# ZackHodari/morgana

Measured on AMD Instinct MI355X. Metric: acoustic frames/sec (fwd+bwd+step), F0Model 600->1, batch 256x1000, higher is better.
Workload: dtype bf16

## Files before the change

### morgana_amd/csrc/gemm_bf16_big.hip

```cpp
#include "common.h"
#include "phone_front.h"
#include "expand_reduce.h"

#include <type_traits>

typedef __bf16 bfv8 __attribute__((ext_vector_type(8)));
typedef __bf16 bfv4 __attribute__((ext_vector_type(4)));


#define MG_ZERO_ELEMS 16384
__device__ uint16_t g_zero_row[MG_ZERO_ELEMS];

__device__ __forceinline__ void glds16(const uint16_t* src, unsigned char* lds_wave_base) {
    const unsigned lds_off = (unsigned)(unsigned long long)((__attribute__((address_space(3))) unsigned char*)lds_wave_base);
    const unsigned lds_uni = __builtin_amdgcn_readfirstlane(lds_off);
    unsigned keep;
    asm volatile("s_mov_b32 %0, m0\n\ts_mov_b32 m0, %2\n\ts_nop 0\n\tglobal_load_lds_dwordx4 %1, off\n\ts_mov_b32 m0, %0"
                 : "=&s"(keep)
                 : "v"(src), "s"(lds_uni)
                 : "memory");
}


#define WAIT_VM_BARRIER(N) asm volatile("s_waitcnt vmcnt(" #N ")\n\ts_barrier" ::: "memory")
#define WAIT_LGKM_BARRIER() asm volatile("s_waitcnt lgkmcnt(0)\n\ts_barrier" ::: "memory")

MG_STAMP_DECL(g_stamps_nt);

#define NT_BIG_LDS(BN_) (((BN_) == 256 ? 4 : 6) * (256 * 64 + (BN_) * 64))
template <int BN, int EPI, int X3 = 0>
__device__ __forceinline__ void gemm_nt_big_body(unsigned char* __restrict__ smem, const unsigned block_id, const uint16_t* __restrict__ A,
                                                 int lda, const int32_t* __restrict__ rows, int64_t M, int K, const uint16_t* __restrict__ Bm,
                                                 int ldb, int N, const float* __restrict__ bias_in, const uint16_t* __restrict__ H, int ldh,
                                                 const int32_t* __restrict__ h_rows, void* __restrict__ Cv_in, int ldc, int tiles_m, int tiles_n,
                                                 int c_f32, float* __restrict__ colsum = nullptr, int wt = 0) {
    const float* bias = bias_in;
    void* Cv = Cv_in;
    constexpr int BM = 256;
    constexpr int WAVES_N = BN / 64;
    constexpr int WAVES_M = 8 / WAVES_N;
    constexpr int WM = BM / WAVES_M;
    constexpr int TM = WM / 32, TN = 2;
    constexpr int A_BYTES = BM * 64, B_BYTES = BN * 64;
    constexpr int STAGE = A_BYTES + B_BYTES;
    constexpr int GA = BM / 16 / 8;
    constexpr int GB = BN / 16 / 8;
    constexpr int NL = GA + GB;
    constexpr int NS = (BN == 256) ? 4 : 6;

    static_assert(NS * STAGE == NT_BIG_LDS(BN), "LDS size helper");

    unsigned tile_id = block_id;
    int my_pass = 0;
    if (X3 == 2) {
        const unsigned per_pass = (unsigned)((tiles_m + 7) / 8) * 8u * (unsigned)tiles_n;
        my_pass = (int)(block_id / per_pass);
        tile_id = block_id - (unsigned)my_pass * per_pass;
    }
    const int xcd = tile_id & 7, jj = tile_id >> 3;
    const int tile_n = jj % tiles_n;
    const int tile_m = (jj / tiles_n) * 8 + xcd;
    if (tile_m >= tiles_m) return;

    const int tid = threadIdx.x, lane = tid & 63;
    const int wave = __builtin_amdgcn_readfirstlane(tid >> 6);
#ifdef MG_STAMPS
    unsigned long long ts0, ts1 = 0, ts2, ts3, tr0, tr1, ta, tb, sum_wait = 0, sum_issue = 0;
    MG_STAMP(ts0);
    MG_STAMP_REAL(tr0);
#endif
    const int wm0 = (wave / WAVES_N) * WM, wn0 = (wave % WAVES_N) * 64;
    const int64_t m0 = (int64_t)tile_m * BM;
    const int n0 = tile_n * BN;
    const int n_kp = (K + 31) / 32;
    const int n_kt = X3 == 1 ? 3 * n_kp : n_kp;
    const int a_lo = lda >> 1, b_lo = ldb >> 1;
    if (X3 == 2) {
        if (my_pass > 0) bias = nullptr;
        Cv = reinterpret_cast<float*>(Cv) + (size_t)my_pass * (size_t)M * ldc;
    }

    const uint16_t* asrc[GA];
    const uint16_t* bsrc[GB];
#pragma unroll
    for (int i = 0; i < GA; ++i) {
        const int row = (wave * GA + i) * 16 + (lane >> 2);
        const int c = (lane & 3) ^ ((row >> 2) & 3);
        const int64_t m = m0 + row;
        const uint16_t* p = g_zero_row;
        if (m < M) {
            if (rows) {
                const int r = rows[m];
                if (r >= 0) p = A + (size_t)r * lda;
            } else {
                p = A + (size_t)m * lda;
            }
        }
        asrc[i] = p + c * 8;
    }
#pragma unroll
    for (int i = 0; i < GB; ++i) {
        const int row = (wave * GB + i) * 16 + (lane >> 2);
        const int c = (lane & 3) ^ ((row >> 2) & 3);
        const int n = n0 + row;
        bsrc[i] = (n < N ? Bm + (size_t)n * ldb : g_zero_row) + c * 8;
    }

    auto issue = [&](int kt) {
        unsigned char* st = smem + (kt % NS) * STAGE;
        int ka = kt * 32, kb = kt * 32;
        if (X3) {
            const int pass = X3 == 2 ? my_pass : kt % 3, w = (X3 == 2 ? kt : kt / 3) * 32;
            ka = w + (pass == 2 ? a_lo : 0);
            kb = w + (pass == 1 ? b_lo : 0);
        }
#pragma unroll
        for (int i = 0; i < GA; ++i) glds16(asrc[i] + ka, st + (wave * GA + i) * 1024);
#pragma unroll
        for (int i = 0; i < GB; ++i) glds16(bsrc[i] + kb, st + A_BYTES + (wave * GB + i) * 1024);
    };

    f32x16 acc[TM][TN];
#pragma unroll
    for (int i = 0; i < TM; ++i)
#pragma unroll
        for (int j = 0; j < TN; ++j)
#pragma unroll
            for (int r = 0; r < 16; ++r) acc[i][j][r] = 0.f;

    const int lr = lane & 31, lh = lane >> 5;
    int aoff[TM], boff[TN];
#pragma unroll
    for (int i = 0; i < TM; ++i) {
        const int row = wm0 + i * 32 + lr;
        aoff[i] = row * 64 + ((lh ^ ((row >> 2) & 3)) << 4);
    }
#pragma unroll
    for (int j = 0; j < TN; ++j) {
        const int row = wn0 + j * 32 + lr;
        boff[j] = A_BYTES + row * 64 + ((lh ^ ((row >> 2) & 3)) << 4);
    }

#pragma unroll
    for (int p = 0; p < NS - 1; ++p)
// ... 697 lines not shown
                    }
                    const bfv2 h01 = bfv2{(__bf16)v[0], (__bf16)v[1]}, h23 = bfv2{(__bf16)v[2], (__bf16)v[3]};
                    const u32x2_t pk = u32x2_t{__builtin_bit_cast(unsigned int, h01), __builtin_bit_cast(unsigned int, h23)};
                    if (X3) {
                        const bfv2 l01 = bfv2{(__bf16)(v[0] - (float)h01[0]), (__bf16)(v[1] - (float)h01[1])};
                        const bfv2 l23 = bfv2{(__bf16)(v[2] - (float)h23[0]), (__bf16)(v[3] - (float)h23[1])};
                        pk_lo[X3 ? j : 0][q] = u32x2_t{__builtin_bit_cast(unsigned int, l01), __builtin_bit_cast(unsigned int, l23)};
                    }
                    const int chunk = 4 * j + q;
                    *reinterpret_cast<u32x2_t*>(patch + lr * SP + ((chunk ^ (lr & 7)) << 4) + 8 * lh) = pk;
                }
            store_rows(i, 0);
            if (X3) {
#pragma unroll
                for (int j = 0; j < TN; ++j)
#pragma unroll
                    for (int q = 0; q < 4; ++q)
                        *reinterpret_cast<u32x2_t*>(patch + lr * SP + (((4 * j + q) ^ (lr & 7)) << 4) + 8 * lh) = pk_lo[X3 ? j : 0][q];
                store_rows(i, ldc >> 1);
            }
        }
        MG_STAMP(tb);
        MG_STAMP_ADD(sum_epi, tb, ta);
    }
    };
    if (lag) run_tiles(std::true_type{}); else run_tiles(std::false_type{});
#ifdef MG_STAMPS
    MG_STAMP(ts2);
    asm volatile("s_waitcnt vmcnt(0)" ::: "memory");
    MG_STAMP(ts3);
    MG_STAMP_REAL(tr1);
    const int sb = block_id;
    MG_STAMP_STORE(g_stamps_ntp, sb, wave, lane, 0, ts0);
    MG_STAMP_STORE(g_stamps_ntp, sb, wave, lane, 1, ts1);
    MG_STAMP_STORE(g_stamps_ntp, sb, wave, lane, 2, ts2);
    MG_STAMP_STORE(g_stamps_ntp, sb, wave, lane, 3, ts3);
    MG_STAMP_STORE(g_stamps_ntp, sb, wave, lane, 4, tr0);
    MG_STAMP_STORE(g_stamps_ntp, sb, wave, lane, 5, tr1);
    MG_STAMP_STORE(g_stamps_ntp, sb, wave, lane, 6, sum_wait);
    MG_STAMP_STORE(g_stamps_ntp, sb, wave, lane, 7, sum_epi);
#endif
}

template <int BN, int EPI, bool STAG, int BK, int MODE = 0>
__global__ __launch_bounds__(512) void gemm_nt_persist_kernel(const uint16_t* __restrict__ A, int lda, const int32_t* __restrict__ rows,
                                                              int64_t M, int K, const uint16_t* __restrict__ Bm, int ldb, int N,
                                                              const float* __restrict__ bias, uint16_t* __restrict__ C, int ldc,
                                                              int tiles_m, int tiles_n, int probe) {
    __shared__ __attribute__((aligned(16))) unsigned char smem[ntp_lds_bytes<BN, BK, MODE>()];
    gemm_nt_persist_body<BN, EPI, STAG, BK, MODE>(smem, blockIdx.x, gridDim.x, A, lda, rows, M, K, Bm, ldb, N, bias, C, ldc, tiles_m, tiles_n,
                                                  probe);
}

template <int EPI, int BMV = 256, int X3 = 0, int BK = 32>
__global__ __launch_bounds__(512) void phone_front_gemm_kernel(unsigned side_blocks, int wave_ints, PhoneFrontArgs pf, const uint16_t* __restrict__ A, int lda,
                                                               int64_t M, int K, const uint16_t* __restrict__ Bm, int ldb, int N,
                                                               const float* __restrict__ bias, uint16_t* __restrict__ C, int ldc, int tiles_m,
                                                               int tiles_n, int wt) {
    static_assert(ntp_lds_bytes<256, BK, 0>() == ntp_lds_bytes<256, 32, 0>(), "the front's jobs were sized for this LDS block");
    __shared__ __attribute__((aligned(16))) unsigned char smem[ntp_lds_bytes<256, BK, 0>()];
    if (blockIdx.x < side_blocks) {
        if (pf.lds_ints > 0) {
            if (wave_ints > 0)
                phone_front_wave_jobs(pf, (int)blockIdx.x * 8 + (int)(threadIdx.x >> 6), (int)side_blocks * 8,
                                      reinterpret_cast<int*>(smem) + (threadIdx.x >> 6) * wave_ints);
            else
                phone_front_block<512>(pf, blockIdx.x, side_blocks, reinterpret_cast<int*>(smem));
        }
        return;
    }
    if (pf.probe & 8) return;
    gemm_nt_persist_body<256, EPI, false, BK, 0, BMV, X3>(smem, blockIdx.x - side_blocks, gridDim.x - side_blocks, A, lda, nullptr, M, K, Bm, ldb, N, bias, C,
                                                     ldc, tiles_m, tiles_n, 0, wt);
}

#define WG_ROWS_MAX 4096
#define WG_STAGES(TKW_) (((TKW_) == 5 || (TKW_) == 4) ? 4 : 3)
MG_STAMP_DECL(g_stamps_wg);

#define WG_BIG_PX(TKW_) ((64 * (TKW_) * 2 + 255) / 256 * 256)
#define WG_BIG_LDS(TKW_) (WG_STAGES(TKW_) * (32 * 256 + 32 * WG_BIG_PX(TKW_)) + WG_ROWS_MAX * 4)
#define WG_STAGES_NW(TKW_, NW_) (((NW_) == 2 && (TKW_) == 5) ? 3 : WG_STAGES(TKW_))
#define WG_BIG_LDS_NW(TKW_, NW_) (WG_STAGES_NW(TKW_, NW_) * (32 * 256 * (NW_) + 32 * WG_BIG_PX(TKW_)) + WG_ROWS_MAX * 4)
template <int TKW, bool DYR = false, int NW = 1, int X3 = 0, bool WT = false>
__device__ __forceinline__ void wgrad_big_body(unsigned char* __restrict__ smem, const unsigned block_id, const uint16_t* __restrict__ dY,
                                               int lddy, const uint16_t* __restrict__ A, int lda, const int32_t* __restrict__ rows, int64_t M,
                                               int N, int K, int m_chunk, float* __restrict__ slab, float* __restrict__ bslab, int64_t sstride,
                                               int xcd_group, const int32_t* __restrict__ dy_rows = nullptr) {
    static_assert(!X3 || !DYR, "X3: no gathered dY form");
    static_assert(NW == 1 || (NW == 2 && (TKW == 4 || TKW == 5)), "the 256-wide n tile goes with a k half (256 or 320 columns)");
    constexpr int BNT = 128 * NW, BKT = 64 * TKW;
    constexpr int KH = (TKW == 5 || TKW == 4) ? 2 : 1;
    constexpr int WK = KH == 2 ? 2 : 4;
    constexpr int TNW = BNT / 32 / (8 / WK);
    constexpr int TKT = BKT / WK / 32;
    constexpr int PY = BNT * 2, PX = WG_BIG_PX(TKW);
    constexpr int XC = BKT * 2 / 16;
    constexpr int Y_BYTES = 32 * PY, X_BYTES = 32 * PX;
    constexpr int STAGE = Y_BYTES + X_BYTES;
    constexpr int NX = X_BYTES / 1024 / 8;
    constexpr int NY = Y_BYTES / 1024 / 8;
    constexpr int NLW = NY + NX;
    static_assert(X_BYTES % 8192 == 0, "whole pieces per wave");
    constexpr bool NATIVE = X3 == 2;
    static_assert(!NATIVE || WG_STAGES_NW(TKW, NW) == 4, "native pair planes: the tiles whose ring has four slots");
    constexpr int NSTG = NATIVE ? 2 : WG_STAGES_NW(TKW, NW);
    constexpr int SLOT = NATIVE ? 2 * STAGE : STAGE;
    constexpr int LDS_BYTES = NSTG * SLOT + WG_ROWS_MAX * 4 * (DYR ? 2 : 1);

    static_assert(LDS_BYTES == WG_BIG_LDS_NW(TKW, NW) + (DYR ? WG_ROWS_MAX * 4 : 0) && LDS_BYTES <= 160 * 1024, "LDS size helper");
    int* row_lds = reinterpret_cast<int*>(smem + NSTG * SLOT);
    int* dyrow_lds = row_lds + WG_ROWS_MAX;

    const int tid = threadIdx.x, lane = tid & 63;
    const int wave = __builtin_amdgcn_readfirstlane(tid >> 6);
#ifdef MG_STAMPS
    unsigned long long ts0, ts1 = 0, ts2, ts3, tr0, tr1, ta, tb, sum_wait = 0, sum_issue = 0;
    MG_STAMP(ts0);
    MG_STAMP_REAL(tr0);
#endif
    const int wn0 = (wave / WK) * (TNW * 32);
    const int wk0 = (wave % WK) * (TKT * 32);
    const int tiles = (N / BNT) * KH;
    int tile, s;
    if (xcd_group) {
        tile = (block_id >> 3) % tiles;
        s = (block_id / (8 * tiles)) * 8 + (block_id & 7);
    } else {
        tile = block_id % tiles;
        s = block_id / tiles;
    }
    const int n0 = (tile / KH) * BNT;
    const int kh = tile % KH, k0 = kh * BKT;
    const int64_t m_lo = (int64_t)s * m_chunk;
    const int64_t m_hi = min(M, m_lo + (int64_t)m_chunk);
    const int n_rows = m_hi > m_lo ? (int)(m_hi - m_lo) : 0;

    for (int i = tid; i < m_chunk; i += 512) {
        int r = -1;
        if (i < n_rows) r = rows ? rows[m_lo + i] : (int)(m_lo + i);
        row_lds[i] = r;
        if (DYR) dyrow_lds[i] = i < n_rows ? dy_rows[m_lo + i] : -1;
    }
    __syncthreads();

    int y_row[NY], y_c[NY];
#pragma unroll
    for (int i = 0; i < NY; ++i) {
        const int byte = (wave * NY + i) * 1024 + lane * 16;
        y_row[i] = byte / PY;
        y_c[i] = ((byte % PY) >> 4) ^ ((y_row[i] & 3) << 2);
    }
    int x_row[NX], x_off[NX];
#pragma unroll
    for (int i = 0; i < NX; ++i) {
        const int byte = (wave * NX + i) * 1024 + lane * 16;
        x_row[i] = byte / PX;
        const int cpos = (byte % PX) >> 4;
        const int src = cpos ^ ((x_row[i] & 3) << 2);
        x_off[i] = src < XC ? k0 + src * 8 : -1;
    }

    const int n_steps1 = (n_rows + 31) / 32;
    auto issue = [&](int step_all) {
        unsigned char* st = smem + (step_all % NSTG) * SLOT;
        int step = step_all, y_plane = 0, a_plane = 0;
        if (NATIVE) {
#pragma unroll
            for (int pl = 0; pl < 2; ++pl) {
#pragma unroll
                for (int i = 0; i < NY; ++i) {
                    const int ml = step * 32 + y_row[i];
                    const uint16_t* p = (ml < n_rows) ? dY + (size_t)(m_lo + ml) * lddy + pl * (lddy >> 1) + n0 + y_c[i] * 8 : g_zero_row;
                    glds16(p, st + pl * STAGE + (wave * NY + i) * 1024);
                }
                int rn[NX];
#pragma unroll
                for (int i = 0; i < NX; ++i) rn[i] = row_lds[step * 32 + x_row[i]];
#pragma unroll
                for (int i = 0; i < NX; ++i) {
                    const uint16_t* p = (rn[i] >= 0 && x_off[i] >= 0) ? A + (size_t)rn[i] * lda + pl * (lda >> 1) + x_off[i] : g_zero_row;
                    glds16(p, st + pl * STAGE + Y_BYTES + (wave * NX + i) * 1024);
                }
            }
            return;
        }
        if (X3) {
            step = step_all / 3;
            const int pass = step_all - 3 * step;
            y_plane = pass == 1 ? (lddy >> 1) : 0;
            a_plane = pass == 2 ? (lda >> 1) : 0;
        }
#pragma unroll
        for (int i = 0; i < NY; ++i) {
            if (DYR) {
                const int ry = dyrow_lds[step * 32 + y_row[i]];
                const uint16_t* p = ry >= 0 ? dY + (size_t)ry * lddy + n0 + y_c[i] * 8 : g_zero_row;
                glds16(p, st + (wave * NY + i) * 1024);
            } else {
                const int ml = step * 32 + y_row[i];
                const uint16_t* p = (ml < n_rows) ? dY + (size_t)(m_lo + ml) * lddy + y_plane + n0 + y_c[i] * 8 : g_zero_row;
                glds16(p, st + (wave * NY + i) * 1024);
            }
        }
        int rr[NX];
#pragma unroll
        for (int i = 0; i < NX; ++i) rr[i] = row_lds[step * 32 + x_row[i]];
#pragma unroll
// ... 128 lines not shown
        }
        if (bias_valu && tid < BNT) {
#pragma unroll 8
            for (int r = 0; r < 32; ++r) {
                const int cpos = (tid >> 3) ^ ((r & 3) << 2);
                bsum += mg_bf2f(*reinterpret_cast<const uint16_t*>(st + r * PY + (cpos << 4) + ((tid & 7) << 1)));
            }
        }
    }

#ifdef MG_STAMPS
    MG_STAMP(ts2);
#endif
    const int lr = lane & 31, lh = lane >> 5;
    float* out = slab + (size_t)s * sstride;
#pragma unroll
    for (int i = 0; i < TNW; ++i) {
#pragma unroll
        for (int j = 0; j < TKT; ++j) {
            const int col = k0 + wk0 + j * 32 + lr;
            if (col >= K) continue;
#pragma unroll
            for (int r = 0; r < 16; ++r) {
                const int row = n0 + wn0 + i * 32 + (r & 3) + 8 * (r >> 2) + 4 * lh;
                if (row < N) mg_store_sel(WT, &out[(size_t)row * K + col], acc[i][j][r]);
            }
        }
    }
    if (bias_valu && tid < BNT && n0 + tid < N) mg_store_sel(WT, &bslab[(size_t)s * sstride + n0 + tid], bsum);
    if ((bias_free || bias_extra) && lr == 0) {
#pragma unroll
        for (int i = 0; i < TNW; ++i) {
#pragma unroll
            for (int r = 0; r < 16; ++r) {
                const int row = n0 + wn0 + i * 32 + (r & 3) + 8 * (r >> 2) + 4 * lh;
                const float v = bias_free ? acc[i][TKT - 1][r] : accb[kExtraBias ? i : 0][r];
                if (row < N) mg_store_sel(WT, &bslab[(size_t)s * sstride + row], v);
            }
        }
    }
#ifdef MG_STAMPS
    asm volatile("s_waitcnt vmcnt(0)" ::: "memory");
    MG_STAMP(ts3);
    MG_STAMP_REAL(tr1);
    const int sb = block_id;
    MG_STAMP_STORE(g_stamps_wg, sb, wave, lane, 0, ts0);
    MG_STAMP_STORE(g_stamps_wg, sb, wave, lane, 1, ts1);
    MG_STAMP_STORE(g_stamps_wg, sb, wave, lane, 2, ts2);
    MG_STAMP_STORE(g_stamps_wg, sb, wave, lane, 3, ts3);
    MG_STAMP_STORE(g_stamps_wg, sb, wave, lane, 4, tr0);
    MG_STAMP_STORE(g_stamps_wg, sb, wave, lane, 5, tr1);
    MG_STAMP_STORE(g_stamps_wg, sb, wave, lane, 6, sum_wait);
    MG_STAMP_STORE(g_stamps_wg, sb, wave, lane, 7, sum_issue);
#endif
}

template <int TKW, int NW = 1, int X3 = 0>
__global__ __launch_bounds__(512) void wgrad_big_kernel(const uint16_t* __restrict__ dY, int lddy, const uint16_t* __restrict__ A, int lda,
                                                        const int32_t* __restrict__ rows, int64_t M, int N, int K, int m_chunk,
                                                        float* __restrict__ slab, float* __restrict__ bslab, int64_t sstride, int xcd_group) {
    __shared__ __attribute__((aligned(16))) unsigned char smem[WG_BIG_LDS_NW(TKW, NW)];
    wgrad_big_body<TKW, false, NW, X3>(smem, blockIdx.x, dY, lddy, A, lda, rows, M, N, K, m_chunk, slab, bslab, sstride, xcd_group);
}

template <int TKW, int NW = 1>
__global__ __launch_bounds__(512) void wgrad_big_rows_kernel(const uint16_t* __restrict__ dY, int lddy, const int32_t* __restrict__ dy_rows,
                                                             const uint16_t* __restrict__ A, int lda, const int32_t* __restrict__ rows, int64_t M,
                                                             int N, int K, int m_chunk, float* __restrict__ slab, float* __restrict__ bslab,
                                                             int64_t sstride, int xcd_group) {
    __shared__ __attribute__((aligned(16))) unsigned char smem[WG_BIG_LDS_NW(TKW, NW) + WG_ROWS_MAX * 4];
    wgrad_big_body<TKW, true, NW>(smem, blockIdx.x, dY, lddy, A, lda, rows, M, N, K, m_chunk, slab, bslab, sstride, xcd_group, dy_rows);
}

template <int TKW, int BN, int X3 = 0>
__global__ __launch_bounds__(512) void wgrad_dgrad_pair_kernel(unsigned wg_blocks, const uint16_t* __restrict__ dY, int lddy,
                                                               const uint16_t* __restrict__ A, int lda, int64_t M, int N, int K, int m_chunk,
                                                               float* __restrict__ slab, float* __restrict__ bslab, int64_t sstride,
                                                               int xcd_group, const uint16_t* __restrict__ WT, int ldwt,
                                                               const uint16_t* __restrict__ H, int ldh, void* __restrict__ dX, int lddx,
                                                               int tiles_m, int tiles_n, unsigned nt_blocks, ExpandReduceArgs xr, int riders,
                                                               float* __restrict__ colsum, int wt) {
    constexpr int LDS = WG_BIG_LDS(TKW) > NT_BIG_LDS(BN) ? WG_BIG_LDS(TKW) : NT_BIG_LDS(BN);
    __shared__ __attribute__((aligned(16))) unsigned char smem[LDS];
    if (blockIdx.x < wg_blocks) {
        constexpr int WX3 = (X3 && WG_STAGES(TKW) == 4) ? 2 : X3;
        if (wt) wgrad_big_body<TKW, false, 1, WX3, true>(smem, blockIdx.x, dY, lddy, A, lda, nullptr, M, N, K, m_chunk, slab, bslab, sstride, xcd_group);
        else wgrad_big_body<TKW, false, 1, WX3, false>(smem, blockIdx.x, dY, lddy, A, lda, nullptr, M, N, K, m_chunk, slab, bslab, sstride, xcd_group);
    }
    else if (blockIdx.x < wg_blocks + nt_blocks)
        gemm_nt_big_body<BN, EPI_SIGMOID_GRAD, X3>(smem, blockIdx.x - wg_blocks, dY, lddy, nullptr, M, N, WT, ldwt, K, nullptr, H, ldh, nullptr, dX,
                                                   lddx, tiles_m, tiles_n, 0, colsum, wt);
    else
        mg_expand_reduce_rider<512>(xr, (int)(blockIdx.x - wg_blocks - nt_blocks), riders, smem);
}


static bool big16(const void* p) { return ((uintptr_t)p % 16) == 0; }

int mg_try_nt_big(const uint16_t* A, int lda, const int32_t* rows, int64_t M, int K, const uint16_t* Bm, int ldb, int N,
                  const float* bias, const uint16_t* H, int ldh, const int32_t* h_rows, void* C, int ldc, int c_f32, int epi,
                  hipStream_t st) {
    if (M < 2048 || lda % 64 != 0 || ldb % 64 != 0 || lda > MG_ZERO_ELEMS - 64 || ldb > MG_ZERO_ELEMS - 64) return 0;
    if (N % 128 != 0 || ldc < N || ldc % 8 != 0 || !big16(A) || !big16(Bm) || !big16(C)) return 0;
    if (EPI_IS_GRAD(epi) && (!H || ldh % 8 != 0 || ldh < N)) return 0;
    if (ldc != N || lda < (K + 63) / 64 * 64 || ldb < (K + 63) / 64 * 64) return 0;
    const int ab = g_mg_tuning[MG_TUNE_AB];
    if (ab == 98 && M < 32768) return 0;
    bool wide = (N % 256 == 0);
    if (wide && ab != 97 && (ab == 99 || mg_ceil_div(M, 256) * (N / 256) < 128)) wide = false;
    const int bn = wide ? 256 : 128;
    const int tiles_n = N / bn;
    const int64_t tiles_m = mg_ceil_div(M, 256);
    const int64_t blocks = mg_ceil_div(tiles_m, 8) * 8 * tiles_n;
    if (blocks >= 2147483647LL || tiles_m >= 2147483647LL) return 0;
    const int n_kt = (K + 31) / 32;
    if (!c_f32 && !EPI_IS_GRAD(epi) && n_kt >= 5 && M < 2147483647LL && 32 % tiles_n == 0 && g_mg_tuning[MG_TUNE_FORM] != 6) {
        int64_t g = 256;
        while (mg_ceil_div(blocks, g) > NTP_MAX_TILES(bn)) g += 256;
        if (g > blocks) g = mg_ceil_div(blocks, 8 * tiles_n) * 8 * tiles_n;
        dim3 pgrid((unsigned)g), pblock(512);
#define LAUNCH_NTP(BN_, EPI_, STAG_, BK_) hipLaunchKernelGGL((gemm_nt_persist_kernel<BN_, EPI_, STAG_, BK_>), pgrid, pblock, 0, st, A, lda, rows, M, K, Bm, ldb, N, bias, (uint16_t*)C, ldc, (int)tiles_m, tiles_n, probe)
        const bool deep = g_mg_tuning[MG_TUNE_FORM] != 3;
#ifdef MG_EXPERIMENTS
        const int form = (epi == EPI_BIAS || epi == EPI_BIAS_SIGMOID) ? g_mg_tuning[MG_TUNE_FORM] : 0;
        const int probe = form >= 256 ? form - 256 : form >= 32 ? form - 32 : 0;
        if (wide && (form == 5 || form == 11)) {
            const int pr = form == 11 ? 32 : 0;
            if (epi == EPI_BIAS) hipLaunchKernelGGL((gemm_nt_persist_kernel<256, EPI_BIAS, false, 32, 2>), pgrid, pblock, 0, st, A, lda, rows, M, K, Bm, ldb, N, bias, (uint16_t*)C, ldc, (int)tiles_m, tiles_n, pr);
            else hipLaunchKernelGGL((gemm_nt_persist_kernel<256, EPI_BIAS_SIGMOID, false, 32, 2>), pgrid, pblock, 0, st, A, lda, rows, M, K, Bm, ldb, N, bias, (uint16_t*)C, ldc, (int)tiles_m, tiles_n, pr);
            return 1;
        }
        if (wide && (form == 9 || form == 10 || form == 12 || form == 13)) {
            hipLaunchKernelGGL((gemm_nt_persist_kernel<256, EPI_BIAS_SIGMOID, false, 32, 5>), pgrid, pblock, 0, st, A, lda, rows, M, K, Bm, ldb, N, bias, (uint16_t*)C, ldc, (int)tiles_m, tiles_n, form == 9 ? 16 : form == 10 ? 24 : form == 12 ? 23 : 23 + 64);
            return 1;
        }
        if (wide && form == 2) {
            if (epi == EPI_BIAS) hipLaunchKernelGGL((gemm_nt_persist_kernel<256, EPI_BIAS, false, 32, 1>), pgrid, pblock, 0, st, A, lda, rows, M, K, Bm, ldb, N, bias, (uint16_t*)C, ldc, (int)tiles_m, tiles_n, probe);
            else hipLaunchKernelGGL((gemm_nt_persist_kernel<256, EPI_BIAS_SIGMOID, false, 32, 1>), pgrid, pblock, 0, st, A, lda, rows, M, K, Bm, ldb, N, bias, (uint16_t*)C, ldc, (int)tiles_m, tiles_n, probe);
            return 1;
        }
        if (wide && form == 4) {
            if (epi == EPI_BIAS) LAUNCH_NTP(256, EPI_BIAS, true, 32); else LAUNCH_NTP(256, EPI_BIAS_SIGMOID, true, 32);
            return 1;
        }
#else
        const int probe = 0;
#endif
#define NTP_WIDE(EPI_) LAUNCH_NTP(256, EPI_, false, 32)
#define NTP_DEEP(EPI_) LAUNCH_NTP(128, EPI_, false, 64)
#define NTP_HALF(EPI_) LAUNCH_NTP(128, EPI_, false, 32)
        if (wide) MG_SWITCH_FWD_EPI(epi, NTP_WIDE);
        else if (deep) MG_SWITCH_FWD_EPI(epi, NTP_DEEP);
        else MG_SWITCH_FWD_EPI(epi, NTP_HALF);
#undef NTP_WIDE
#undef NTP_DEEP
#undef NTP_HALF
#undef LAUNCH_NTP
        return 1;
    }
    dim3 grid((unsigned)blocks), block(512);
#define LAUNCH_NT(BN_, EPI_) hipLaunchKernelGGL((gemm_nt_big_kernel<BN_, EPI_>), grid, block, 0, st, A, lda, rows, M, K, Bm, ldb, N, bias, H, ldh, h_rows, C, ldc, (int)tiles_m, tiles_n, c_f32)
#define NT_WIDE(EPI_) LAUNCH_NT(256, EPI_)
#define NT_HALF(EPI_) LAUNCH_NT(128, EPI_)
    if (wide) {
        if (EPI_IS_GRAD(epi)) MG_SWITCH_GRAD_EPI(epi, NT_WIDE);
        else MG_SWITCH_FWD_EPI(epi, NT_WIDE);
    } else {
        if (EPI_IS_GRAD(epi)) MG_SWITCH_GRAD_EPI(epi, NT_HALF);
        else MG_SWITCH_FWD_EPI(epi, NT_HALF);
    }
#undef NT_WIDE
#undef NT_HALF
#undef LAUNCH_NT
    return 1;
// ... 69 lines not shown
            hipLaunchKernelGGL((wgrad_big_rows_kernel<8>), grid, block, 0, st, dY, lddy, dy_rows, A, lda, rows, M, N, K, m_chunk, slab, bslab,
                               sstride, xg);
        return 1;
    }
    const bool ksplit = wgrad_ksplit(M, N, lda);
    dim3 grid((unsigned)((N / 128) * (ksplit ? 2 : 1) * S)), block(512);
    int xcd_group = (rows == nullptr && S % 8 == 0) ? 1 : 0;
    if (g_mg_tuning[MG_TUNE_WGRAD_ORDER] == 1) xcd_group = 0;
    if (g_mg_tuning[MG_TUNE_WGRAD_ORDER] == 2 && S % 8 == 0) xcd_group = 1;
    if (!ksplit && lda == 512 && N % 256 == 0 && g_mg_tuning[MG_TUNE_AB] != 91)
        hipLaunchKernelGGL((wgrad_big_kernel<4, 2>), grid, block, 0, st, dY, lddy, A, lda, rows, M, N, K, m_chunk, slab, bslab, sstride, xcd_group);
    else if (ksplit && lda == 512)
        hipLaunchKernelGGL((wgrad_big_kernel<4>), grid, block, 0, st, dY, lddy, A, lda, rows, M, N, K, m_chunk, slab, bslab, sstride, xcd_group);
    else if (ksplit)
        hipLaunchKernelGGL((wgrad_big_kernel<5>), grid, block, 0, st, dY, lddy, A, lda, rows, M, N, K, m_chunk, slab, bslab, sstride, xcd_group);
    else if (lda == 640 && N % 256 == 0 && g_mg_tuning[MG_TUNE_AB] != 91)
        hipLaunchKernelGGL((wgrad_big_kernel<5, 2>), grid, block, 0, st, dY, lddy, A, lda, rows, M, N, K, m_chunk, slab, bslab, sstride, xcd_group);
    else if (lda == 640)
        hipLaunchKernelGGL((wgrad_big_kernel<10>), grid, block, 0, st, dY, lddy, A, lda, rows, M, N, K, m_chunk, slab, bslab, sstride, xcd_group);
    else
        hipLaunchKernelGGL((wgrad_big_kernel<8>), grid, block, 0, st, dY, lddy, A, lda, rows, M, N, K, m_chunk, slab, bslab, sstride, xcd_group);
    return 1;
}

int mg_launch_phone_front_gemm(const PhoneFrontArgs& pf, const uint16_t* A, int lda, int64_t M, int K, const uint16_t* Bm, int ldb, int N,
                               const float* bias, uint16_t* C, int ldc, int epi, hipStream_t st) {
    if (g_mg_tuning[MG_TUNE_AB] == 66 || g_mg_tuning[MG_TUNE_FORM] != 0) return 0;
    if (M < 2048 || M >= 2147483647LL || lda % 64 != 0 || ldb % 64 != 0 || lda > MG_ZERO_ELEMS - 64 || ldb > MG_ZERO_ELEMS - 64) return 0;
    if (N % 256 != 0 || ldc != N || !big16(A) || !big16(Bm) || !big16(C)) return 0;
    if (lda < (K + 63) / 64 * 64 || ldb < (K + 63) / 64 * 64 || (K + 31) / 32 < 5) return 0;
    if (epi != EPI_BIAS && epi != EPI_BIAS_SIGMOID) return 0;
    const int tiles_n = N / 256;
    if (32 % tiles_n != 0) return 0;
    constexpr int LDS_INTS = ntp_lds_bytes<256, 32, 0>() / 4;
    const int64_t wave_ints_need = phone_front_wave_ints(pf.B, pf.P, pf.T, pf.extra);
    const int wave_ints = (g_mg_tuning[MG_TUNE_AB] != 94 && 8 * wave_ints_need <= LDS_INTS) ? (int)wave_ints_need : 0;
    int bmv = 256;
    if (wave_ints > 0 && g_mg_tuning[MG_TUNE_AB] != 95 && mg_ceil_div(mg_ceil_div(M, 192), 8) * 8 * tiles_n <= 224) bmv = 192;
    const int64_t tiles_m = mg_ceil_div(M, bmv);
    const int64_t blocks = mg_ceil_div(tiles_m, 8) * 8 * tiles_n;
    if (blocks > 224) return 0;
    const int64_t g = mg_ceil_div(blocks, 8 * tiles_n) * 8 * tiles_n;
    const int side = (int)((256 - g) / 8 * 8);
    if (side < 32) return 0;
    if (phone_front_lds_ints(pf.B, pf.P, pf.T, pf.extra) > LDS_INTS) return 0;
    PhoneFrontArgs a = pf;
    a.lds_ints = LDS_INTS;
#ifdef MG_EXPERIMENTS
    if (g_mg_tuning[MG_TUNE_AB] == 67) a.lds_ints = 0;
    if (g_mg_tuning[MG_TUNE_AB] >= 70 && g_mg_tuning[MG_TUNE_AB] < 85) a.probe = g_mg_tuning[MG_TUNE_AB] - 70;
#endif
    dim3 grid((unsigned)(side + g)), block(512);
#define LAUNCH_PFG(EPI_, BMV_, BK_)                                                                                                             \
    hipLaunchKernelGGL((phone_front_gemm_kernel<EPI_, BMV_, 0, BK_>), grid, block, 0, st, (unsigned)side, wave_ints, a, A, lda, M, K, Bm, ldb, N, bias, C, \
                       ldc, (int)tiles_m, tiles_n, wt)
    const int wt = (mg_wt_mask() & MG_WT_FWD) ? 1 : 0;
    const bool deep64 = g_mg_tuning[MG_TUNE_AB] == 88 && lda % 64 == 0 && ldb % 64 == 0;
    if (epi == EPI_BIAS) {
        if (bmv == 192) { if (deep64) LAUNCH_PFG(EPI_BIAS, 192, 64); else LAUNCH_PFG(EPI_BIAS, 192, 32); }
        else { if (deep64) LAUNCH_PFG(EPI_BIAS, 256, 64); else LAUNCH_PFG(EPI_BIAS, 256, 32); }
    } else {
        if (bmv == 192) { if (deep64) LAUNCH_PFG(EPI_BIAS_SIGMOID, 192, 64); else LAUNCH_PFG(EPI_BIAS_SIGMOID, 192, 32); }
        else { if (deep64) LAUNCH_PFG(EPI_BIAS_SIGMOID, 256, 64); else LAUNCH_PFG(EPI_BIAS_SIGMOID, 256, 32); }
    }
#undef LAUNCH_PFG
    return 1;
}

int mg_launch_wgrad_dgrad_pair(const uint16_t* dY, int lddy, const uint16_t* A, int lda, int64_t M, int N, int K, const uint16_t* WT, int ldwt,
                               uint16_t* dX, int lddx, float* slab, int64_t sstride, size_t slab_floats, int* S_out, hipStream_t st,
                               const ExpandReduceArgs* rider, int x3, float* colsum) {
    if (g_mg_tuning[MG_TUNE_AB] == 65) return 0;
    int S = 0, m_chunk = 0;
    const int pl = x3 ? 2 : 1;
    if (x3 && (lddy % 2 || lda % 2 || ldwt % 2 || lddx % 2 || !colsum)) return 0;
    const int lda_p = lda / pl, lddy_p = lddy / pl, ldwt_p = ldwt / pl;
    if (N != 128 || K != 512 || lda_p != 512 || lddx != pl * K || mg_wgrad_big_plan(M, N, K, lda_p, lddy_p, &S, &m_chunk) <= 0) return 0;
    if (lddy_p % 64 != 0 || ldwt_p % 64 != 0 || lddy > MG_ZERO_ELEMS - 64 || ldwt > MG_ZERO_ELEMS - 64 || lddy_p < 128 || ldwt_p < 128) return 0;
    if (!big16(dY) || !big16(A) || !big16(WT) || !big16(dX)) return 0;
    const int tiles_n = K / 256;
    const int64_t tiles_m = mg_ceil_div(M, 256);
    const bool ksplit = wgrad_ksplit(M, N, lda_p);
    const int kt = ksplit ? 2 : 1;
    auto fits = [&](int S_, int chunk_) {
        const int64_t s_real = mg_ceil_div(M, chunk_);
        for (int x = 0; x < 8; ++x) {
            const int64_t nt_x = (tiles_m > x ? mg_ceil_div(tiles_m - x, 8) : 0) * tiles_n;
            int64_t wg_x = 0;
            for (int b = x; b < S_; b += 8) wg_x += b < s_real ? kt : 0;
            if (nt_x + wg_x > 32) return false;
        }
        return true;
    };
    bool found = false;
    for (int cand = S; cand >= 48 / kt && !found; cand -= 8) {
        const int chunk_ = cand == S ? m_chunk : (int)mg_align_up((size_t)mg_ceil_div(M, cand), 32);
        if (chunk_ > WG_ROWS_MAX) break;
        const int S_ = (int)mg_align_up((size_t)mg_ceil_div(M, chunk_), 8);
        if (S_ > S || !fits(S_, chunk_)) continue;
        found = true;
        S = S_;
        m_chunk = chunk_;
    }
    if (!found) return 0;
    if ((size_t)S * (size_t)sstride > slab_floats) return 0;
    const unsigned nt_blocks = (unsigned)(mg_ceil_div(tiles_m, 8) * 8 * tiles_n);
    ExpandReduceArgs xr{};
    int riders = 0;
    if (rider) {
        xr = *rider;
        const int64_t by_frames = mg_ceil_div(xr.M, 2048), by_chunks = mg_ceil_div(mg_ceil_div(xr.n, 16) - xr.first_chunk, 2);
        riders = (int)(by_frames > by_chunks ? by_frames : by_chunks);
        if (riders < 1) riders = 1;
        if (riders > 1024) riders = 1024;
    }
    const int wt = (mg_wt_mask() & MG_WT_PAIR) ? 1 : 0;
    if (x3) {
        if (ksplit)
            hipLaunchKernelGGL((wgrad_dgrad_pair_kernel<4, 256, 1>), dim3((unsigned)(2 * S) + nt_blocks + riders), dim3(512), 0, st, (unsigned)(2 * S),
                               dY, lddy, A, lda, M, N, K, m_chunk, slab, (float*)nullptr, sstride, 1, WT, ldwt, A, lda, (void*)dX, lddx, (int)tiles_m,
                               tiles_n, nt_blocks, xr, riders, colsum, wt);
        else
            hipLaunchKernelGGL((wgrad_dgrad_pair_kernel<8, 256, 1>), dim3((unsigned)S + nt_blocks + riders), dim3(512), 0, st, (unsigned)S, dY, lddy,
                               A, lda, M, N, K, m_chunk, slab, (float*)nullptr, sstride, 1, WT, ldwt, A, lda, (void*)dX, lddx, (int)tiles_m, tiles_n,
                               nt_blocks, xr, riders, colsum, wt);
        *S_out = S;
        return 1;
    }
    if (ksplit)
        hipLaunchKernelGGL((wgrad_dgrad_pair_kernel<4, 256>), dim3((unsigned)(2 * S) + nt_blocks + riders), dim3(512), 0, st, (unsigned)(2 * S), dY,
                           lddy, A, lda, M, N, K, m_chunk, slab, slab + (int64_t)N * K, sstride, 1, WT, ldwt, A, lda, (void*)dX, lddx, (int)tiles_m,
                           tiles_n, nt_blocks, xr, riders, (float*)nullptr, wt);
    else
        hipLaunchKernelGGL((wgrad_dgrad_pair_kernel<8, 256>), dim3((unsigned)S + nt_blocks + riders), dim3(512), 0, st, (unsigned)S, dY, lddy, A, lda,
                           M, N, K, m_chunk, slab, slab + (int64_t)N * K, sstride, 1, WT, ldwt, A, lda, (void*)dX, lddx, (int)tiles_m, tiles_n,
                           nt_blocks, xr, riders, (float*)nullptr, wt);
    *S_out = S;
    return 1;
}

int mg_launch_nt_persist_x3(const PhoneFrontArgs* pf, const uint16_t* A, int lda, int64_t M, int K, const uint16_t* Bm, int ldb, int N,
                            const float* bias, uint16_t* C, int ldc, int epi, hipStream_t st, int* front_rode) {
    if (front_rode) *front_rode = 0;
    if (M < 1 || M >= 2147483647LL || lda % 128 != 0 || ldb % 128 != 0 || lda > MG_ZERO_ELEMS - 64 || ldb > MG_ZERO_ELEMS - 64) return 0;
    const int pa = lda / 2, pb = ldb / 2;
    if (N % 256 != 0 || ldc != 2 * N || !big16(A) || !big16(Bm) || !big16(C)) return 0;
    if (pa < (K + 63) / 64 * 64 || pb < (K + 63) / 64 * 64 || (K + 31) / 32 < 2) return 0;
    if (epi != EPI_BIAS && epi != EPI_BIAS_SIGMOID) return 0;
    const int tiles_n = N / 256;
    if (32 % tiles_n != 0) return 0;
    constexpr int LDS_INTS = ntp_lds_bytes<256, 32, 0>() / 4;
    PhoneFrontArgs a{};
    int side = 0, wave_ints = 0, bmv = 256;
    int64_t g = 0, tiles_m = 0;
    if (pf && g_mg_tuning[MG_TUNE_AB] != 66) {
        const int64_t wave_ints_need = phone_front_wave_ints(pf->B, pf->P, pf->T, pf->extra);
        wave_ints = (8 * wave_ints_need <= LDS_INTS) ? (int)wave_ints_need : 0;
        if (wave_ints > 0 && mg_ceil_div(mg_ceil_div(M, 192), 8) * 8 * tiles_n <= 224) bmv = 192;
        tiles_m = mg_ceil_div(M, bmv);
        const int64_t blocks = mg_ceil_div(tiles_m, 8) * 8 * tiles_n;
        g = mg_ceil_div(blocks, 8 * tiles_n) * 8 * tiles_n;
        side = (int)((256 - g) / 8 * 8);
        if (blocks <= 224 && side >= 32 && phone_front_lds_ints(pf->B, pf->P, pf->T, pf->extra) <= LDS_INTS) {
            a = *pf;
            a.lds_ints = LDS_INTS;
            if (front_rode) *front_rode = 1;
        } else {
            side = 0;
        }
    }
    if (side == 0) {
        bmv = 256;
        wave_ints = 0;
        tiles_m = mg_ceil_div(M, 256);
        const int64_t blocks = mg_ceil_div(tiles_m, 8) * 8 * tiles_n;
        g = 256;
        while (mg_ceil_div(blocks, g) > NTP_MAX_TILES(256)) g += 256;
        if (g > blocks) g = mg_ceil_div(blocks, 8 * tiles_n) * 8 * tiles_n;
    }
    dim3 grid((unsigned)(side + g)), block(512);
#define LAUNCH_PFG3(EPI_, BMV_, X3_, BK_)                                                                                                        \
    hipLaunchKernelGGL((phone_front_gemm_kernel<EPI_, BMV_, X3_, BK_>), grid, block, 0, st, (unsigned)side, wave_ints, a, A, lda, M, K, Bm, ldb, N, bias, C, \
                       ldc, (int)tiles_m, tiles_n, wt)
    const int wt = ((mg_wt_mask() & MG_WT_FWD) && side > 0) ? 1 : 0;
    const int ab3 = g_mg_tuning[MG_TUNE_AB];
    if (ab3 == 87) {
        if (epi == EPI_BIAS) { if (bmv == 192) LAUNCH_PFG3(EPI_BIAS, 192, 1, 64); else LAUNCH_PFG3(EPI_BIAS, 256, 1, 64); }
        else { if (bmv == 192) LAUNCH_PFG3(EPI_BIAS_SIGMOID, 192, 1, 64); else LAUNCH_PFG3(EPI_BIAS_SIGMOID, 256, 1, 64); }
        return 1;
    }
    const bool passes = ab3 == 89;
    if (epi == EPI_BIAS) {
        if (bmv == 192) { if (passes) LAUNCH_PFG3(EPI_BIAS, 192, 1, 32); else LAUNCH_PFG3(EPI_BIAS, 192, 2, 32); }
        else { if (passes) LAUNCH_PFG3(EPI_BIAS, 256, 1, 32); else LAUNCH_PFG3(EPI_BIAS, 256, 2, 32); }
    } else {
        if (bmv == 192) { if (passes) LAUNCH_PFG3(EPI_BIAS_SIGMOID, 192, 1, 32); else LAUNCH_PFG3(EPI_BIAS_SIGMOID, 192, 2, 32); }
        else { if (passes) LAUNCH_PFG3(EPI_BIAS_SIGMOID, 256, 1, 32); else LAUNCH_PFG3(EPI_BIAS_SIGMOID, 256, 2, 32); }
    }
#undef LAUNCH_PFG3
    return 1;
}

int mg_launch_nt_big_x3_f32(const uint16_t* A, int lda, int64_t M, int K, const uint16_t* Bm, int ldb, int N, const float* bias, float* C,
                            int ldc, int epi, hipStream_t st, int parts) {
    if (parts == 3) {
        if (M < 1 || lda % 128 != 0 || ldb % 128 != 0 || lda > MG_ZERO_ELEMS - 64 || ldb > MG_ZERO_ELEMS - 64 || epi != EPI_BIAS) return 0;
        if (N % 128 != 0 || ldc != N || !big16(A) || !big16(Bm) || !big16(C) || lda / 2 < (K + 63) / 64 * 64 || ldb / 2 < (K + 63) / 64 * 64) return 0;
        const int64_t tm = mg_ceil_div(M, 256);
        const int tn = N / 128;
        const int64_t per_pass = mg_ceil_div(tm, 8) * 8 * tn;
        if (3 * per_pass >= 2147483647LL) return 0;
        hipLaunchKernelGGL((gemm_nt_big_kernel<128, EPI_BIAS, 2>), dim3((unsigned)(3 * per_pass)), dim3(512), 0, st, A, lda, (const int32_t*)nullptr, M, K,
                           Bm, ldb, N, bias, (const uint16_t*)nullptr, 0, (const int32_t*)nullptr, (void*)C, ldc, (int)tm, tn, 1);
        return 1;
    }
    if (parts != 1) return 0;
    if (M < 1 || lda % 128 != 0 || ldb % 128 != 0 || lda > MG_ZERO_ELEMS - 64 || ldb > MG_ZERO_ELEMS - 64) return 0;
    const int pa = lda / 2, pb = ldb / 2;
// ... 31 lines not shown
```

### morgana_amd/csrc/runtime.hip

```cpp
#include "common.h"

#include <stdarg.h>
#include <string.h>

#include <thread>
#include <vector>

static thread_local char g_error[512] = "";

void mg_set_error(const char* fmt, ...) {
    va_list ap;
    va_start(ap, fmt);
    vsnprintf(g_error, sizeof(g_error), fmt, ap);
    va_end(ap);
}

int g_mg_tuning[MG_TUNING_KEYS] = {0};

extern "C" {

static bool tuning_allowed(int key, int value) {
#ifdef MG_EXPERIMENTS
    (void)key;
    (void)value;
    return true;
#else
    switch (key) {
        case MG_TUNE_FORM: return value == 0 || value == 3 || value == 6 || value == 7 || value == 12 || value == 13 || value == 14 || value == 16;
        case MG_TUNE_GRU_HANDOFF: return value >= 0 && value <= 7;
        case MG_TUNE_PERSISTENT: return value >= 0 && value <= 2;
        case MG_TUNE_WGRAD_SPLITS: return value >= 0;
        case MG_TUNE_WGRAD_ORDER: return value >= 0 && value <= 3;
        case MG_TUNE_LSTM_BWD_STACK: return value >= 0 && value <= 3;
        case MG_TUNE_AB: return value == 0 || value == 65 || value == 66 || value == 85 || value == 86 || value == 87 || value == 88 || value == 89 || value == 90 || value == 91 || value == 92 || value == 93 || value == 94 || value == 95 || value == 96 || value == 97 || value == 98 || value == 99;
        default: return false;
    }
#endif
}

int mg_set_tuning(int key, int value) {
    MG_CHECK_ARG(key >= 0 && key < MG_TUNING_KEYS, "mg_set_tuning: key %d not in 0..%d", key, MG_TUNING_KEYS - 1);
    MG_CHECK_ARG(tuning_allowed(key, value),
                 "mg_set_tuning: key %d does not take value %d in the product library (experiments and timing probes are compiled into the "
                 "lab builds only: make -C morgana_amd/csrc lab)", key, value);
    g_mg_tuning[key] = value;
    return MG_OK;
}

const char* mg_last_error(void) { return g_error; }

int mg_version(void) { return 1; }

const char* mg_build_arch(void) { return "gfx950"; }

int mg_host_pack(const void* const* srcs, const int64_t* bytes, int count, void* dst, int64_t dst_bytes, int threads) {
    MG_CHECK_ARG(srcs && bytes && dst && count > 0 && threads > 0 && threads <= 64, "mg_host_pack: bad arguments (count=%d threads=%d)", count,
                 threads);
    int64_t total = 0;
    for (int i = 0; i < count; ++i) {
        MG_CHECK_ARG(bytes[i] >= 0 && (bytes[i] == 0 || srcs[i]), "mg_host_pack: bad piece %d", i);
        total += bytes[i];
    }
    MG_CHECK_ARG(total <= dst_bytes, "mg_host_pack: %lld bytes do not fit the destination's %lld", (long long)total, (long long)dst_bytes);
    if (total == 0) return MG_OK;
    auto work = [&](int64_t lo, int64_t hi) {
        int64_t at = 0;
        for (int i = 0; i < count && at < hi; ++i) {
            const int64_t b = bytes[i], p_lo = lo > at ? lo : at, p_hi = hi < at + b ? hi : at + b;
            if (p_hi > p_lo) memcpy((char*)dst + p_lo, (const char*)srcs[i] + (p_lo - at), (size_t)(p_hi - p_lo));
            at += b;
        }
    };
    int n = threads;
    if (total < (int64_t)n * (1 << 20)) n = (int)(total >> 20) + 1;
    if (n <= 1) {
        work(0, total);
        return MG_OK;
    }
    const int64_t per = ((total + n - 1) / n + 63) / 64 * 64;
    std::vector<std::thread> pool;
    for (int t = 1; t < n; ++t) pool.emplace_back(work, (int64_t)t * per < total ? (int64_t)t * per : total, (int64_t)(t + 1) * per < total ? (int64_t)(t + 1) * per : total);
    work(0, per < total ? per : total);
    for (auto& th : pool) th.join();
    return MG_OK;
}

}
```

Before: 2.556 billion.

## Place wgrad splits and dgrad tiles as contiguous row ranges per XCD

```diff
diff --git a/morgana_amd/csrc/gemm_bf16_big.hip b/morgana_amd/csrc/gemm_bf16_big.hip
--- a/morgana_amd/csrc/gemm_bf16_big.hip
+++ b/morgana_amd/csrc/gemm_bf16_big.hip
@@ -1,6 +1,7 @@
 #include "common.h"
 #include "phone_front.h"
 #include "expand_reduce.h"
+#include "pair_place.h"
 
 #include <type_traits>
 
@@ -33,7 +34,7 @@
                                                  int lda, const int32_t* __restrict__ rows, int64_t M, int K, const uint16_t* __restrict__ Bm,
                                                  int ldb, int N, const float* __restrict__ bias_in, const uint16_t* __restrict__ H, int ldh,
                                                  const int32_t* __restrict__ h_rows, void* __restrict__ Cv_in, int ldc, int tiles_m, int tiles_n,
-                                                 int c_f32, float* __restrict__ colsum = nullptr, int wt = 0) {
+                                                 int c_f32, float* __restrict__ colsum = nullptr, int wt = 0, int place = 0) {
     const float* bias = bias_in;
     void* Cv = Cv_in;
     constexpr int BM = 256;
@@ -58,8 +59,13 @@
         tile_id = block_id - (unsigned)my_pass * per_pass;
     }
     const int xcd = tile_id & 7, jj = tile_id >> 3;
-    const int tile_n = jj % tiles_n;
-    const int tile_m = (jj / tiles_n) * 8 + xcd;
+    int tile_n = jj % tiles_n;
+    int tile_m = (jj / tiles_n) * 8 + xcd;
+    if (place == MG_PAIR_ROW_RANGE) {
+        const MgPairWork pw = mg_pair_place(MG_PAIR_ROW_RANGE, tile_id, 0u, 8, 1, tiles_m, tiles_n);
+        tile_n = pw.tile_n;
+        tile_m = pw.body == MG_PAIR_DGRAD ? pw.tile_m : tiles_m;
+    }
     if (tile_m >= tiles_m) return;
 
     const int tid = threadIdx.x, lane = tid & 63;
@@ -923,11 +929,11 @@
 #define WG_BIG_LDS(TKW_) (WG_STAGES(TKW_) * (32 * 256 + 32 * WG_BIG_PX(TKW_)) + WG_ROWS_MAX * 4)
 #define WG_STAGES_NW(TKW_, NW_) (((NW_) == 2 && (TKW_) == 5) ? 3 : WG_STAGES(TKW_))
 #define WG_BIG_LDS_NW(TKW_, NW_) (WG_STAGES_NW(TKW_, NW_) * (32 * 256 * (NW_) + 32 * WG_BIG_PX(TKW_)) + WG_ROWS_MAX * 4)
-template <int TKW, bool DYR = false, int NW = 1, int X3 = 0, bool WT = false>
+template <int TKW, bool DYR = false, int NW = 1, int X3 = 0, bool WT = false, bool PLACE = false>
 __device__ __forceinline__ void wgrad_big_body(unsigned char* __restrict__ smem, const unsigned block_id, const uint16_t* __restrict__ dY,
                                                int lddy, const uint16_t* __restrict__ A, int lda, const int32_t* __restrict__ rows, int64_t M,
                                                int N, int K, int m_chunk, float* __restrict__ slab, float* __restrict__ bslab, int64_t sstride,
-                                               int xcd_group, const int32_t* __restrict__ dy_rows = nullptr) {
+                                               int xcd_group, const int32_t* __restrict__ dy_rows = nullptr, int n_splits = 0) {
     static_assert(!X3 || !DYR, "X3: no gathered dY form");
     static_assert(NW == 1 || (NW == 2 && (TKW == 4 || TKW == 5)), "the 256-wide n tile goes with a k half (256 or 320 columns)");
     constexpr int BNT = 128 * NW, BKT = 64 * TKW;
@@ -964,7 +970,11 @@
     const int wk0 = (wave % WK) * (TKT * 32);
     const int tiles = (N / BNT) * KH;
     int tile, s;
-    if (xcd_group) {
+    if (PLACE && xcd_group == 2) {
+        const MgPairWork pw = mg_pair_place(MG_PAIR_ROW_RANGE, block_id, (unsigned)(tiles * n_splits), n_splits, tiles, 0, 1);
+        tile = pw.khalf;
+        s = pw.split;
+    } else if (xcd_group) {
         tile = (block_id >> 3) % tiles;
         s = (block_id / (8 * tiles)) * 8 + (block_id & 7);
     } else {
@@ -1259,14 +1269,17 @@
                                                                float* __restrict__ colsum, int wt) {
     constexpr int LDS = WG_BIG_LDS(TKW) > NT_BIG_LDS(BN) ? WG_BIG_LDS(TKW) : NT_BIG_LDS(BN);
     __shared__ __attribute__((aligned(16))) unsigned char smem[LDS];
+    const int place = xcd_group == 2 ? MG_PAIR_ROW_RANGE : MG_PAIR_ROUND_ROBIN;
     if (blockIdx.x < wg_blocks) {
         constexpr int WX3 = (X3 && WG_STAGES(TKW) == 4) ? 2 : X3;
-        if (wt) wgrad_big_body<TKW, false, 1, WX3, true>(smem, blockIdx.x, dY, lddy, A, lda, nullptr, M, N, K, m_chunk, slab, bslab, sstride, xcd_group);
-        else wgrad_big_body<TKW, false, 1, WX3, false>(smem, blockIdx.x, dY, lddy, A, lda, nullptr, M, N, K, m_chunk, slab, bslab, sstride, xcd_group);
+        constexpr int KT = (TKW == 5 || TKW == 4) ? 2 : 1;
+        const int n_splits = (int)(wg_blocks / KT);
+        if (wt) wgrad_big_body<TKW, false, 1, WX3, true, true>(smem, blockIdx.x, dY, lddy, A, lda, nullptr, M, N, K, m_chunk, slab, bslab, sstride, xcd_group, nullptr, n_splits);
+        else wgrad_big_body<TKW, false, 1, WX3, false, true>(smem, blockIdx.x, dY, lddy, A, lda, nullptr, M, N, K, m_chunk, slab, bslab, sstride, xcd_group, nullptr, n_splits);
     }
     else if (blockIdx.x < wg_blocks + nt_blocks)
         gemm_nt_big_body<BN, EPI_SIGMOID_GRAD, X3>(smem, blockIdx.x - wg_blocks, dY, lddy, nullptr, M, N, WT, ldwt, K, nullptr, H, ldh, nullptr, dX,
-                                                   lddx, tiles_m, tiles_n, 0, colsum, wt);
+                                                   lddx, tiles_m, tiles_n, 0, colsum, wt, place);
     else
         mg_expand_reduce_rider<512>(xr, (int)(blockIdx.x - wg_blocks - nt_blocks), riders, smem);
 }
@@ -1502,26 +1515,10 @@
     const int64_t tiles_m = mg_ceil_div(M, 256);
     const bool ksplit = wgrad_ksplit(M, N, lda_p);
     const int kt = ksplit ? 2 : 1;
-    auto fits = [&](int S_, int chunk_) {
-        const int64_t s_real = mg_ceil_div(M, chunk_);
-        for (int x = 0; x < 8; ++x) {
-            const int64_t nt_x = (tiles_m > x ? mg_ceil_div(tiles_m - x, 8) : 0) * tiles_n;
-            int64_t wg_x = 0;
-            for (int b = x; b < S_; b += 8) wg_x += b < s_real ? kt : 0;
-            if (nt_x + wg_x > 32) return false;
-        }
-        return true;
-    };
-    bool found = false;
-    for (int cand = S; cand >= 48 / kt && !found; cand -= 8) {
-        const int chunk_ = cand == S ? m_chunk : (int)mg_align_up((size_t)mg_ceil_div(M, cand), 32);
-        if (chunk_ > WG_ROWS_MAX) break;
-        const int S_ = (int)mg_align_up((size_t)mg_ceil_div(M, chunk_), 8);
-        if (S_ > S || !fits(S_, chunk_)) continue;
-        found = true;
-        S = S_;
-        m_chunk = chunk_;
-    }
+    int place = MG_PAIR_ROUND_ROBIN;
+    const bool found = mg_pair_choose_splits(M, S, m_chunk, kt, (int)tiles_m, tiles_n, WG_ROWS_MAX,
+                                             g_mg_tuning[MG_TUNE_AB] == 60 ? MG_PAIR_ROUND_ROBIN : MG_PAIR_ROW_RANGE, &S, &m_chunk, &place);
+    const int xg = place == MG_PAIR_ROW_RANGE ? 2 : 1;
     if (!found) return 0;
     if ((size_t)S * (size_t)sstride > slab_floats) return 0;
     const unsigned nt_blocks = (unsigned)(mg_ceil_div(tiles_m, 8) * 8 * tiles_n);
@@ -1538,22 +1535,22 @@
     if (x3) {
         if (ksplit)
             hipLaunchKernelGGL((wgrad_dgrad_pair_kernel<4, 256, 1>), dim3((unsigned)(2 * S) + nt_blocks + riders), dim3(512), 0, st, (unsigned)(2 * S),
-                               dY, lddy, A, lda, M, N, K, m_chunk, slab, (float*)nullptr, sstride, 1, WT, ldwt, A, lda, (void*)dX, lddx, (int)tiles_m,
+                               dY, lddy, A, lda, M, N, K, m_chunk, slab, (float*)nullptr, sstride, xg, WT, ldwt, A, lda, (void*)dX, lddx, (int)tiles_m,
                                tiles_n, nt_blocks, xr, riders, colsum, wt);
         else
             hipLaunchKernelGGL((wgrad_dgrad_pair_kernel<8, 256, 1>), dim3((unsigned)S + nt_blocks + riders), dim3(512), 0, st, (unsigned)S, dY, lddy,
-                               A, lda, M, N, K, m_chunk, slab, (float*)nullptr, sstride, 1, WT, ldwt, A, lda, (void*)dX, lddx, (int)tiles_m, tiles_n,
+                               A, lda, M, N, K, m_chunk, slab, (float*)nullptr, sstride, xg, WT, ldwt, A, lda, (void*)dX, lddx, (int)tiles_m, tiles_n,
                                nt_blocks, xr, riders, colsum, wt);
         *S_out = S;
         return 1;
     }
     if (ksplit)
         hipLaunchKernelGGL((wgrad_dgrad_pair_kernel<4, 256>), dim3((unsigned)(2 * S) + nt_blocks + riders), dim3(512), 0, st, (unsigned)(2 * S), dY,
-                           lddy, A, lda, M, N, K, m_chunk, slab, slab + (int64_t)N * K, sstride, 1, WT, ldwt, A, lda, (void*)dX, lddx, (int)tiles_m,
+                           lddy, A, lda, M, N, K, m_chunk, slab, slab + (int64_t)N * K, sstride, xg, WT, ldwt, A, lda, (void*)dX, lddx, (int)tiles_m,
                            tiles_n, nt_blocks, xr, riders, (float*)nullptr, wt);
     else
         hipLaunchKernelGGL((wgrad_dgrad_pair_kernel<8, 256>), dim3((unsigned)S + nt_blocks + riders), dim3(512), 0, st, (unsigned)S, dY, lddy, A, lda,
-                           M, N, K, m_chunk, slab, slab + (int64_t)N * K, sstride, 1, WT, ldwt, A, lda, (void*)dX, lddx, (int)tiles_m, tiles_n,
+                           M, N, K, m_chunk, slab, slab + (int64_t)N * K, sstride, xg, WT, ldwt, A, lda, (void*)dX, lddx, (int)tiles_m, tiles_n,
                            nt_blocks, xr, riders, (float*)nullptr, wt);
     *S_out = S;
     return 1;
diff --git a/morgana_amd/csrc/pair_place.h b/morgana_amd/csrc/pair_place.h
--- /dev/null
+++ b/morgana_amd/csrc/pair_place.h
@@ -0,0 +1,88 @@
+#pragma once
+#include <stdint.h>
+
+#if defined(__HIPCC__)
+#define MG_PLACE_FN __host__ __device__ __forceinline__
+#else
+#define MG_PLACE_FN static inline
+#endif
+
+#define MG_PAIR_ROUND_ROBIN 0
+#define MG_PAIR_ROW_RANGE 1
+
+#define MG_PAIR_WGRAD 0
+#define MG_PAIR_DGRAD 1
+#define MG_PAIR_IDLE 2
+#define MG_PAIR_RIDER 3
+
+struct MgPairWork {
+    int body;
+    int split, khalf;
+    int tile_m, tile_n;
+};
+
+MG_PLACE_FN int mg_pair_tiles_lo(int x, int tiles_m) { return (int)(((int64_t)x * tiles_m + 7) / 8); }
+
+MG_PLACE_FN MgPairWork mg_pair_place(int mode, unsigned block_id, unsigned wg_blocks, int S, int kt, int tiles_m, int tiles_n) {
+    MgPairWork w{MG_PAIR_RIDER, 0, 0, 0, 0};
+    const unsigned x = block_id & 7u;
+    if (block_id < wg_blocks) {
+        const unsigned j = block_id >> 3;
+        w.body = MG_PAIR_WGRAD;
+        w.khalf = (int)(j % (unsigned)kt);
+        if (mode == MG_PAIR_ROW_RANGE) w.split = (int)(x * (unsigned)(S / 8) + j / (unsigned)kt);
+        else w.split = (int)((j / (unsigned)kt) * 8u + x);
+        return w;
+    }
+    const unsigned t = block_id - wg_blocks;
+    const unsigned tiles_pad = (unsigned)((tiles_m + 7) / 8) * 8u;
+    if (t >= tiles_pad * (unsigned)tiles_n) return w;
+    const unsigned j = t >> 3;
+    w.tile_n = (int)(j % (unsigned)tiles_n);
+    int tm, hi;
+    if (mode == MG_PAIR_ROW_RANGE) {
+        tm = mg_pair_tiles_lo((int)x, tiles_m) + (int)(j / (unsigned)tiles_n);
+        hi = mg_pair_tiles_lo((int)x + 1, tiles_m);
+    } else {
+        tm = (int)(j / (unsigned)tiles_n) * 8 + (int)x;
+        hi = tiles_m;
+    }
+    w.tile_m = tm;
+    w.body = tm < hi ? MG_PAIR_DGRAD : MG_PAIR_IDLE;
+    return w;
+}
+
+MG_PLACE_FN int64_t mg_pair_xcd_load(int mode, int x, int S, int kt, int64_t s_real, int tiles_m, int tiles_n) {
+    int64_t nt, wg = 0;
+    if (mode == MG_PAIR_ROW_RANGE) {
+        nt = mg_pair_tiles_lo(x + 1, tiles_m) - mg_pair_tiles_lo(x, tiles_m);
+        for (int s = x * (S / 8); s < (x + 1) * (S / 8); ++s) wg += s < s_real ? kt : 0;
+    } else {
+        nt = tiles_m > x ? (tiles_m - x + 7) / 8 : 0;
+        for (int s = x; s < S; s += 8) wg += s < s_real ? kt : 0;
+    }
+    return nt * tiles_n + wg;
+}
+
+MG_PLACE_FN bool mg_pair_fits(int mode, int64_t M, int S, int m_chunk, int kt, int tiles_m, int tiles_n) {
+    const int64_t s_real = (M + m_chunk - 1) / m_chunk;
+    for (int x = 0; x < 8; ++x)
+        if (mg_pair_xcd_load(mode, x, S, kt, s_real, tiles_m, tiles_n) > 32) return false;
+    return true;
+}
+
+MG_PLACE_FN bool mg_pair_choose_splits(int64_t M, int S_plan, int chunk_plan, int kt, int tiles_m, int tiles_n, int rows_max, int want_mode,
+                                       int* S_out, int* chunk_out, int* mode_out) {
+    for (int cand = S_plan; cand >= 48 / kt; cand -= 8) {
+        const int64_t chunk_ = cand == S_plan ? chunk_plan : ((M + cand - 1) / cand + 31) / 32 * 32;
+        if (chunk_ > rows_max) break;
+        const int64_t S_ = ((M + chunk_ - 1) / chunk_ + 7) / 8 * 8;
+        if (S_ > S_plan || !mg_pair_fits(MG_PAIR_ROUND_ROBIN, M, (int)S_, (int)chunk_, kt, tiles_m, tiles_n)) continue;
+        *S_out = (int)S_;
+        *chunk_out = (int)chunk_;
+        *mode_out = (want_mode == MG_PAIR_ROW_RANGE && mg_pair_fits(MG_PAIR_ROW_RANGE, M, (int)S_, (int)chunk_, kt, tiles_m, tiles_n))
+                        ? MG_PAIR_ROW_RANGE : MG_PAIR_ROUND_ROBIN;
+        return true;
+    }
+    return false;
+}
diff --git a/morgana_amd/csrc/runtime.hip b/morgana_amd/csrc/runtime.hip
--- a/morgana_amd/csrc/runtime.hip
+++ b/morgana_amd/csrc/runtime.hip
@@ -32,7 +32,7 @@
         case MG_TUNE_WGRAD_SPLITS: return value >= 0;
         case MG_TUNE_WGRAD_ORDER: return value >= 0 && value <= 3;
         case MG_TUNE_LSTM_BWD_STACK: return value >= 0 && value <= 3;
-        case MG_TUNE_AB: return value == 0 || value == 65 || value == 66 || value == 85 || value == 86 || value == 87 || value == 88 || value == 89 || value == 90 || value == 91 || value == 92 || value == 93 || value == 94 || value == 95 || value == 96 || value == 97 || value == 98 || value == 99;
+        case MG_TUNE_AB: return value == 0 || value == 60 || value == 65 || value == 66 || value == 85 || value == 86 || value == 87 || value == 88 || value == 89 || value == 90 || value == 91 || value == 92 || value == 93 || value == 94 || value == 95 || value == 96 || value == 97 || value == 98 || value == 99;
         default: return false;
     }
 #endif
```

Result: no change. 2.569 billion, median of 6 (+0.5%).
